# lijrjyan/SDVAR

Measured on AMD Instinct MI355X. Metric: images/s (+ mean accepted tokens/step), VAR-d16 256^2 B=8, d12 draft + d16 verify, per GPU, higher is better.
Workload: dtype f32 (GEMM operands split into 2 fp16 planes to 2^-22, 3 fp16 MFMA products, fp32 accumulate); 1 GPU; BASELINE.json P1: VAR-d16 256^2 B=8/GPU, d12 draft + d16 verify, gamma=2, cfg=1.5 top_k=900 top_p=0.96, acceptance=natural, incl. VQVAE decode (overlapped with the next batch on a 2nd stream); verifier one round behind the draft once gamma = 1; parallelism=1 independent batch shards

## Files before the change

include/sdvar_hip.h:

```cpp
#ifndef SDVAR_HIP_H
#define SDVAR_HIP_H
#include <stdint.h>

#ifdef __cplusplus
extern "C" {
#endif

#define SDVAR_ABI_VERSION 5
#define SDVAR_MAX_STAGES 16

typedef struct sdvar_model sdvar_model_t;
typedef struct sdvar_quant sdvar_quant_t;
typedef struct sdvar_vae sdvar_vae_t;
typedef struct sdvar_vae_enc sdvar_vae_enc_t;

typedef struct {
    int32_t depth;
    int32_t n_stages;
    int32_t patch_nums[SDVAR_MAX_STAGES];
    int32_t vocab;
    int32_t cvae;
    int32_t num_classes;
    int32_t max_batch;
    int32_t max_chunk_stages;
// ... 139 lines not shown
int sdvar_op_quant_nearest(const float* z, int32_t N, const float* codebook, int32_t V, int32_t cvae, float* e2, int64_t* ids, void* stream);
int sdvar_op_conv_planes(const uint16_t* x_planes, uint64_t x_plane_stride, uint64_t x_rows, int32_t x_row0, const uint16_t* w_planes, uint64_t w_plane_stride,
                         int32_t plane_format, const float* w_scale, const float* bias, const float* res, float* out, int32_t B, int32_t H, int32_t W, int32_t N,
                         int32_t Cin, int32_t taps, float* workspace, uint64_t workspace_floats, int32_t force_split, void* stream);
int sdvar_op_conv_planes_ex(const uint16_t* x_planes, uint64_t x_plane_stride, uint64_t x_rows, int32_t x_row0, const uint16_t* w_planes, uint64_t w_plane_stride,
                            int32_t plane_format, const float* w_scale, const float* bias, const float* res, float* out, int32_t B, int32_t H, int32_t W, int32_t N,
                            int32_t Cin, int32_t taps, float* workspace, uint64_t workspace_floats, int32_t force_split, int32_t up_phase, uint64_t w_phase_stride,
                            double* gn_part, float* stats, int32_t* gn_done, void* stream);
int sdvar_op_upconv_weights(const float* w, float* weff, int32_t Cout, int32_t Cin, void* stream);
int sdvar_op_vae_gn_stats(const float* x_rows, int32_t B, int32_t C, int32_t H, int32_t W, double* part_ws, float* stats, void* stream);
int sdvar_op_vae_attn(const float* qkv, float* out, int32_t B, int32_t C, int32_t N, float* workspace, uint64_t ws_floats, int32_t kernel, void* stream);
int sdvar_op_vae_conv_out(const float* x_rows, const float* stats, const float* gamma, const float* beta, const float* w, const float* bias, float* img, int32_t B,
                          int32_t C, int32_t H, int32_t W, float* workspace, void* stream);
int sdvar_debug_set_gemm_cfg(int32_t bm, int32_t split);
int sdvar_debug_set_qkv_fuse(int32_t on);
int sdvar_debug_set_rowblk(int32_t on);
int sdvar_op_gemm_rowblk(const float* x, int32_t ldx, const float* scale, const float* shift, int32_t rows_per_img, int32_t mod_stride, const uint16_t* Xp, uint64_t x_plane_stride,
                         const uint16_t* Wp, uint64_t w_plane_stride, const float* w_scale, const float* bias, float* out, int32_t ldo, uint16_t* out_planes, uint64_t out_plane_stride,
                         int32_t M, int32_t N, int32_t K, int32_t epilogue, const float* res, int32_t ldres, const float* gate, int32_t rows_per_gate, int32_t gate_stride,
                         const float* scale_mul, float* q_out, void* k_cache, void* v_cache, int32_t l, int32_t H, int32_t Lp, int32_t pos0, int32_t kv_fmt, void* stream);
int sdvar_debug_set_variant(const char* name, int32_t value);
int sdvar_debug_get_gemm_cfg(int32_t* out4);
int sdvar_debug_get_conv_cfg(int32_t* out1);
int sdvar_debug_get_conv_plan(int32_t* out4);
int sdvar_debug_plan_gemm(int32_t mode, int32_t M, int32_t N, int32_t K, int32_t flags, int32_t* out4);
int sdvar_debug_set_f16x2_guard(int32_t on);
int sdvar_debug_get_f16x2_guard(uint64_t* out4, int32_t reset);
int sdvar_debug_set_gemm_stamps(uint64_t* stamps);

#define SDVAR_PROF_CLASSES 10
int sdvar_prof_enable(int32_t on);
int sdvar_prof_collect(double* ms , int64_t* launches, double* flops, double* bytes);

int sdvar_op_sdpa_hm(const void* q, const void* k, const void* v, void* out, const int64_t* strides , int32_t dtype , int32_t q_f32,
                     int32_t k_f32, const void* bias, int32_t bias_kind , const int64_t* bias_strides ,
                     const uint8_t* skip_map, int32_t B, int32_t H, int32_t Lq, int32_t Lk, int32_t head_dim, double scale, void* stream);

int sdvar_op_sdpa_hm_lse(const void* q, const void* k, const void* v, void* out, float* lse, const int64_t* strides , int32_t dtype ,
                         int32_t q_f32, int32_t k_f32, const void* bias, int32_t bias_kind ,
                         const int64_t* bias_strides , const uint8_t* skip_map, int32_t B, int32_t H, int32_t Lq, int32_t Lk, int32_t head_dim, double scale,
                         void* stream);
int sdvar_op_sdpa_h_bwd(const void* q, const void* k, const void* v, const void* out, const void* dout, const float* lse, float* delta , void* dq, void* dk,
                        void* dv, const int64_t* strides , int32_t dtype , int32_t q_f32, int32_t k_f32, const void* bias,
                        int32_t bias_kind , const int64_t* bias_strides , const uint8_t* skip_map,
                        int32_t B, int32_t H, int32_t Lq, int32_t Lk, int32_t head_dim, double scale, void* stream);

// ... 66 lines not shown
```

sdvar_amd/csrc/api.hip:

```cpp
#include <math.h>
#include <stdarg.h>
#include <string.h>

#include <vector>

#include "../../include/sdvar_hip.h"
#include "common.h"
#include "gemm_plan.h"

namespace sdvar {

int gemm_f32_nt(const float* X, int ldx, const float* W, const float* bias, float* out, int ldo, int M, int N, int K, int epi,
                const float* res, int ldres, const float* gate, int rows_per_gate, int gate_stride, hipStream_t stream);
struct PendingSplitK { const float* ws; const float* bias; const float* gate; int split, rows_per_gate, gate_stride; };
int ln_modulate(float* x, const float* scale, const float* shift, float* out, uint16_t* outp, size_t ops, int rows, int C, int rows_per_img, int mod_stride, const PendingSplitK* pend, int pfmt, hipStream_t stream);
float* splitk_workspace(size_t* floats);
float* set_splitk_workspace(float* p);
size_t splitk_workspace_floats();
int qk_norm_append(const float* qkv, const float* scale_mul, float* q_out, void* k_cache, void* v_cache, int kv_f16, int R, int l, int H, int Lmax, int pos0, const PendingSplitK* pend, int v_only, hipStream_t stream);
int gemm_f16x2_qkv(const uint16_t* X, size_t xps, const uint16_t* W, size_t wps, const float* wsi, const float* bias, float* out, int ldo, int M, int N, int K,
                   const float* scale_mul, float* q_out, void* k_cache, void* v_cache, int l, int H, int Lp, int pos0, int kv_fmt, int* defer, int* fused, hipStream_t stream);
bool gemm_f16x2_rowblk_ok(int M, int N, int K, int ln, int qkv, bool floor32);
bool gemm_f16x2_rowblk_want(int M, int C, int V, int rows_per_img);
int gemm_f16x2_rowblk(const float* x, int ldx, const float* scale, const float* shift, int rows_per_img, int mod_stride, const uint16_t* X, size_t xps,
// ... 26 lines not shown
int gate_add_bwd(const float* g, const void* y, int ydt, const void* gamma, int gdt, long long gbs, const float* row_scale, void* dy, void* dgamma, int dgamma_rows,
                 float* ws, int B, int L, int C, hipStream_t stream);
long long gate_add_bwd_ws_bytes(int B, int L, int C);
int qknorm_fwd(const void* qkv, int dt, const float* q_bias, const float* v_bias, const float* scale_log, double max_log, float* q, float* k, void* v, int B, int L, int H,
               hipStream_t stream);
int qknorm_bwd(const void* qkv, int dt, const float* q_bias, const float* scale_log, double max_log, const float* dq, const float* dk, const void* dv,
               const long long* strides, void* dqkv, float* dscale_log, float* dq_bias, float* dv_bias, float* ws, int B, int L, int H, hipStream_t stream);
long long qknorm_bwd_ws_bytes(int B, int L, int H);
int cond_lin_fwd(const void* c, int cdt, long long ldc, const void* w, int wdt, const float* b, void* y, int adt, int M, int N, int K, hipStream_t stream);
int cond_lin_bwd(const void* dy, const void* c, int cdt, long long ldc, const void* w, int wdt, void* dc, void* dW, float* db, float* ws, int adt, int M, int N, int K,
                 hipStream_t stream);
long long cond_lin_bwd_ws_bytes(int M, int N, int K);
int embed_fwd(const void* label, int i64, const float* r, double rate, const long long* lvl, const float* xv, long long xbs, long long xrs, const float* class_emb,
              const float* pos_start, const float* W, const float* bias, const float* lvl_emb, const float* pos, void* x, int xdt, float* cond, int B, int T, int L, int first_l,
              int C, int K, int S, int NC1, hipStream_t stream);
int embed_bwd(const void* g, int gdt, const float* gc, const void* label, int i64, const float* r, double rate, const long long* lvl, const float* xv, long long xbs,
              long long xrs, const float* W, float* dpos, float* dpos_start, float* dlvl, float* dclass, float* dbias, float* dW, float* dxv, int xv_rows, float* ws, int B, int T,
              int L, int first_l, int C, int K, int S, int NC1, hipStream_t stream);
long long embed_bwd_ws_bytes(int B, int T, int C, int K);
int optim_grad_stats(const sdvar_optim_tensor_t* ts, int n, const float* grad_scale, const float* found_inf, double max_norm, double beta1, double beta2, void* ws,
                     unsigned long long ws_bytes, hipStream_t stream);
int optim_adamw_step(const sdvar_optim_tensor_t* ts, int n, double beta1, double beta2, double eps, void* ws, unsigned long long ws_bytes, hipStream_t stream);
int attention_f32(const float* q, const void* kc, const void* vc, int kv_f16, float* out, uint16_t* outp, size_t ops, int pfmt, int R, int H, int l, int Lmax, int Ktot, int n_chunk, const int* qbeg, const int* vis, hipStream_t stream);
int gemm_bf16x3_nt(const uint16_t* X, size_t xps, const uint16_t* W, size_t wps, const float* bias, float* out, int ldo, uint16_t* outp, size_t ops,
                   int M, int N, int K, int epi, const float* res, int ldres, const float* gate, int rows_per_gate, int gate_stride, int* defer, hipStream_t stream);
int attention_masked(const float* q, const void* kc, const void* vc, int fmt, const float* bias, float* out, uint16_t* outp, size_t ops, int pfmt, int R, int H, int l,
                     int Lmax, int Ktot, hipStream_t stream);
int attention_sdpa(const float* q, const float* k, const float* v, float* out, const long long* strides, const void* bias, int kind, const long long* bs,
                   const uint8_t* skip, int B, int H, int Lq, int Lk, int head_dim, float scale, hipStream_t stream);
int sdpa_skip_map(const void* bias, int kind, const long long* bs, int Bb, int Hb, int Lq, int Lk, uint8_t* map, hipStream_t stream);
int attention_sdpa_lse(const float* q, const float* k, const float* v, float* out, float* lse, const long long* strides, const void* bias, int kind, const long long* bs,
                       const uint8_t* skip, int B, int H, int Lq, int Lk, int head_dim, float scale, hipStream_t stream);
int attention_sdpa_bwd(const float* q, const float* k, const float* v, const float* out, const float* dout, const float* lse, float* delta, float* dq, float* dk,
                       float* dv, const long long* strides, const void* bias, int kind, const long long* bs, const uint8_t* skip, int B, int H, int Lq, int Lk,
                       int head_dim, float scale, hipStream_t stream);
int attention_sdpa_h(const void* q, const void* k, const void* v, void* out, const long long* strides, int dtype, int B, int H, int Lq, int Lk, int head_dim, double scale,
                     hipStream_t stream);
int attention_sdpa_hm(const void* q, const void* k, const void* v, void* out, const long long* strides, int dtype, int q_f32, int k_f32, const void* bias, int kind,
                      const long long* bs, const uint8_t* skip, int B, int H, int Lq, int Lk, int head_dim, double scale, hipStream_t stream);
int attention_sdpa_hm_lse(const void* q, const void* k, const void* v, void* out, float* lse, const long long* strides, int dtype, int q_f32, int k_f32, const void* bias,
                          int kind, const long long* bs, const uint8_t* skip, int B, int H, int Lq, int Lk, int head_dim, double scale, hipStream_t stream);
int attention_sdpa_h_bwd(const void* q, const void* k, const void* v, const void* out, const void* dout, const float* lse, float* delta, void* dq, void* dk, void* dv,
                         const long long* strides, int dtype, int q_f32, int k_f32, const void* bias, int kind, const long long* bs, const uint8_t* skip, int B, int H,
                         int Lq, int Lk, int head_dim, double scale, hipStream_t stream);
int split_planes(const float* x, uint16_t* planes, int rows, int cols, size_t plane_stride, hipStream_t stream);
int gemm_half_ex(const void* x, const void* w, int dtype, const float* w_scale, const float* bias, float* out, int ldo, void* h_out, void* p_out, const float* res, int ldres,
// ... 1078 lines not shown
int sdvar_debug_plan_gemm(int32_t mode, int32_t M, int32_t N, int32_t K, int32_t flags, int32_t* out4) {
    SDVAR_CHECK_ARG(out4 && mode >= 0 && mode <= 2, "debug_plan_gemm: mode %d", mode);
    SDVAR_CHECK_ARG(M > 0 && N > 0 && K > 0 && K % 32 == 0, "debug_plan_gemm: need K %% 32 == 0 (M=%d N=%d K=%d)", M, N, K);
    const size_t wsf = splitk_workspace_floats();
    const GemmPlan p = mode == 0 ? plan_f32(M, N, K, wsf) : mode == 1 ? plan_bf16x3(M, N, K, wsf) : !(flags & 8) ? plan_f16x2(M, N, K, wsf, flags & 1, flags & 2, flags & 4)
                                                                                                                : plan_f16(M, N, K, wsf, flags & 1, flags & 2, flags & 4);
    out4[0] = p.kernel; out4[1] = p.split; out4[2] = p.tail; out4[3] = p.qkv_fused;
    return SDVAR_OK;
}

int sdvar_debug_get_gemm_cfg(int32_t* out4) {
    SDVAR_CHECK_ARG(out4, "debug_get_gemm_cfg: null");
    int v[4]; debug_get_gemm_cfg_h(v);
    for (int i = 0; i < 4; ++i) out4[i] = v[i];
    return SDVAR_OK;
}

int sdvar_debug_get_conv_cfg(int32_t* out1) {
    SDVAR_CHECK_ARG(out1, "debug_get_conv_cfg: null");
    out1[0] = debug_get_conv_tap_reuse();
    return SDVAR_OK;
}

int sdvar_debug_get_conv_plan(int32_t* out4) {
    SDVAR_CHECK_ARG(out4, "debug_get_conv_plan: null");
    int v[4]; debug_get_conv_plan(v);
    for (int i = 0; i < 4; ++i) out4[i] = v[i];
    return SDVAR_OK;
}

int sdvar_debug_set_f16x2_guard(int32_t on) {
    if (on && !g_guard_cnt) {
        SDVAR_HIP(hipMalloc((void**)&g_guard_cnt, 4 * sizeof(unsigned long long)));
        SDVAR_HIP(hipMemset(g_guard_cnt, 0, 4 * sizeof(unsigned long long)));
    }
    g_guard_on = on != 0;
    return SDVAR_OK;
}

int sdvar_debug_get_f16x2_guard(uint64_t* out4, int32_t reset) {
    SDVAR_CHECK_ARG(out4, "debug_get_f16x2_guard: null");
    for (int i = 0; i < 4; ++i) out4[i] = 0;
    if (!g_guard_cnt) return SDVAR_OK;
    SDVAR_HIP(hipDeviceSynchronize());
    SDVAR_HIP(hipMemcpy(out4, g_guard_cnt, 4 * sizeof(unsigned long long), hipMemcpyDeviceToHost));
    if (reset) SDVAR_HIP(hipMemset(g_guard_cnt, 0, 4 * sizeof(unsigned long long)));
// ... 31 lines not shown
```

sdvar_amd/csrc/attention_f16x2.hip:

```cpp
#include <stdlib.h>

#include "common.h"
#include "gemm_plan.h"

namespace sdvar {

unsigned long long* debug_get_gemm_stamps();

typedef _Float16 f16x8 __attribute__((ext_vector_type(8)));
typedef _Float16 f16x2v __attribute__((ext_vector_type(2)));
typedef uint16_t u16x8 __attribute__((ext_vector_type(8)));
typedef __attribute__((address_space(3))) void* lds_ptr_t;
typedef const __attribute__((address_space(1))) void* glb_ptr_t;

constexpr int ATTH_MAX_CHUNK = 16;
constexpr int AKT = 32;
constexpr int APL = AKT * 64;
constexpr int ANST = 3;

struct AttnHArgs {
    const float* q; const uint16_t* kc; const uint16_t* vc; float* out;
    uint16_t* outp; size_t ops; int pfmt;
    int R, H, l, Lp, Ktot;
    int n_chunk;
    int qbeg[ATTH_MAX_CHUNK + 1];
    int vis[ATTH_MAX_CHUNK];
    unsigned long long* stamps;
};

__device__ __forceinline__ void split8h(const float* v, f16x8& h, f16x8& l) {
#pragma unroll
    for (int e = 0; e < 8; ++e) {
        const float x = clamp_f16_range(v[e]);
        const _Float16 hh = (_Float16)x;
        h[e] = hh; l[e] = (_Float16)(x - (float)hh);
    }
}

typedef short s16x4 __attribute__((ext_vector_type(4)));
__device__ __forceinline__ f16x8 lds_read_tr8(uint32_t addr, int off) {
    typedef __attribute__((address_space(3))) s16x4* lp_t;
    const s16x4 lo = __builtin_amdgcn_ds_read_tr16_b64_v4i16((lp_t)(uintptr_t)(addr + off));
    const s16x4 hi = __builtin_amdgcn_ds_read_tr16_b64_v4i16((lp_t)(uintptr_t)(addr + off + 1024));
    return __builtin_bit_cast(f16x8, __builtin_shufflevector(lo, hi, 0, 1, 2, 3, 4, 5, 6, 7));
}

template <int NKP>
__device__ __forceinline__ void mfma_planes(f32x16& acc, const f16x8* a, const f16x8* b) {
    if (NKP == 2) acc = __builtin_amdgcn_mfma_f32_32x32x16_f16(a[1], b[0], acc, 0, 0, 0);
    acc = __builtin_amdgcn_mfma_f32_32x32x16_f16(a[0], b[1], acc, 0, 0, 0);
// ... 196 lines not shown

    if (wave_active && qi_raw < a.l) {
        const float inv = 1.0f / l_run;
        const size_t obase = ((size_t)r * a.l + qi_raw) * (a.H * 64) + h * 64 + 4 * lh;
#pragma unroll
        for (int g = 0; g < 4; ++g) {
            f32x4 v0, v1;
#pragma unroll
            for (int e = 0; e < 4; ++e) { v0[e] = o0[4 * g + e] * inv; v1[e] = o1[4 * g + e] * inv; }
            if (a.outp) {
                const float u0[4] = {v0[0], v0[1], v0[2], v0[3]}, u1[4] = {v1[0], v1[1], v1[2], v1[3]};
                const int orow = r * a.l + qi_raw, ocol = h * 64 + 4 * lh + 8 * g;
                store_planes4(a.outp, a.ops, kb_index(orow, ocol, a.R * a.l), u0, a.pfmt);
                store_planes4(a.outp, a.ops, kb_index(orow, ocol + 32, a.R * a.l), u1, a.pfmt);
            } else {
                *reinterpret_cast<f32x4*>(a.out + obase + 8 * g) = v0;
                *reinterpret_cast<f32x4*>(a.out + obase + 32 + 8 * g) = v1;
            }
        }
    }
}


template <int NKP, int SCHED>
__global__ __launch_bounds__(512, 2) void attention_f16x2_pp_kernel(AttnHArgs a) {
    extern __shared__ __attribute__((aligned(16))) uint16_t att_sm[];
    constexpr int ASTAGE = 2 * NKP * APL;
    constexpr int PP_NST = SCHED == 0 ? 3 : 2 * SCHED + 2;

    const int tid = threadIdx.x, lane = tid & 63;
    const int wave = __builtin_amdgcn_readfirstlane(tid >> 6);
    const int li = lane & 31, lh = lane >> 5;
    const int qt = blockIdx.x, h = blockIdx.y, r = blockIdx.z;
    const int q0 = qt * 256;
    const int late = wave >> 2;

    const int qi_raw = q0 + wave * 32 + li;
    const int qi = min(qi_raw, a.l - 1);
    int vis_q = a.vis[0];
#pragma unroll 1
    for (int j = 1; j < a.n_chunk; ++j) if (qi >= a.qbeg[j]) vis_q = a.vis[j];
    const int q_last = min(q0 + 255, a.l - 1);
    int kend = a.vis[0];
#pragma unroll 1
    for (int j = 1; j < a.n_chunk; ++j) if (q_last >= a.qbeg[j]) kend = a.vis[j];
    const bool wave_active = (q0 + wave * 32) < a.l;

    f16x8 qp[4][2];
    {
        const float* pq = a.q + (((size_t)r * a.H + h) * a.l + qi) * 64 + 8 * lh;
#pragma unroll
        for (int c = 0; c < 4; ++c) {
            float v[8];
            const f32x4 u0 = *reinterpret_cast<const f32x4*>(pq + 16 * c), u1 = *reinterpret_cast<const f32x4*>(pq + 16 * c + 4);
#pragma unroll
            for (int e = 0; e < 4; ++e) { v[e] = u0[e]; v[4 + e] = u1[e]; }
            split8h(v, qp[c][0], qp[c][1]);
        }
#pragma unroll
        for (int c = 0; c < 4; ++c) { asm volatile("" : "+v"(qp[c][0]), "+v"(qp[c][1])); }
    }

    const size_t head = ((size_t)r * a.H + h) * NKP * (size_t)a.Lp * 64;
    const size_t kps = (size_t)a.Lp * 64;
    const int drow = 8 * (wave & 3) + (lane >> 3);
    const int dchunk = (lane & 7) ^ (late ? 4 * ((drow >> 1) & 1) : ((drow >> 1) & 7));
    const uint32_t ld = (uint32_t)(drow * 64 + 8 * dchunk) * 2u;
    const char* const bsrc = reinterpret_cast<const char*>((late ? a.vc : a.kc) + head);
    const uint32_t lds0 = SDVAR_LDS_ADDR(att_sm);
    auto issue = [&](int t) {
        const uint32_t st = lds0 + (uint32_t)((t % PP_NST) * ASTAGE + (late ? NKP * APL : 0) + (wave & 3) * 512) * 2u;
#pragma unroll
        for (int p = 0; p < NKP; ++p) SDVAR_DMA16(ld, bsrc + (p * kps + (size_t)t * AKT * 64) * 2, st + (uint32_t)(p * APL) * 2u);
    };

    f32x16 o0, o1;
#pragma unroll
    for (int i = 0; i < 16; ++i) { o0[i] = 0.f; o1[i] = 0.f; }
    float M_run = -INFINITY, l_run = 0.f;

    const int swk = (li >> 1) & 7;
    const int vq = (lane >> 2) & 3, vp = lane & 3, vcb = (lane >> 4) & 1;
    const uint32_t koff = (uint32_t)(li * 128), voff0 = (uint32_t)(NKP * APL * 2 + (4 * lh + vq) * 128 + (((vq >> 1) & 1) * 64) + vcb * 32 + vp * 8);
    const int ntiles = (kend + AKT - 1) / AKT;

    f16x8 kf[4][NKP], vf[2][2][NKP];
    auto read_k = [&](int t) {
        const uint32_t sb = lds0 + (uint32_t)((t % PP_NST) * ASTAGE) * 2u;
#pragma unroll
        for (int c = 0; c < 4; ++c)
#pragma unroll
            for (int p = 0; p < NKP; ++p) SDVAR_LDS_RDP(kf[c][p], sb + koff + (uint32_t)(p * APL * 2 + 16 * ((2 * c + lh) ^ swk)));
    };
    auto read_v = [&](int t) {
        const uint32_t sb = lds0 + (uint32_t)((t % PP_NST) * ASTAGE) * 2u;
        const uint32_t sv0 = sb + voff0, sv1 = sv0 ^ 64u;
#pragma unroll
        for (int j = 0; j < 2; ++j)
#pragma unroll
            for (int p = 0; p < NKP; ++p) {
                vf[j][0][p] = lds_read_tr8(sv0, j * 2048 + p * (APL * 2));
                vf[j][1][p] = lds_read_tr8(sv1, j * 2048 + p * (APL * 2));
            }
    };
    auto read_tile = [&](int t) { read_k(t); read_v(t); };
#define SDVAR_PP_SLOT() do { __builtin_amdgcn_sched_barrier(0); __builtin_amdgcn_s_barrier(); __builtin_amdgcn_sched_barrier(0); } while (0)
#ifdef SDVAR_ATT_STAMPS
    unsigned long long stm[5] = {0, 0, 0, 0, 0}, wsr[4] = {0, 0, 0, 0}, wsc[4] = {0, 0, 0, 0};
    wsr[0] = __builtin_amdgcn_s_memrealtime(); wsc[0] = __builtin_amdgcn_s_memtime();
#define SDVAR_PP_STAMP(k) do { if (t == 10) stm[k] = __builtin_amdgcn_s_memtime(); } while (0)
#else
#define SDVAR_PP_STAMP(k) do { } while (0)
#endif

    if constexpr (SCHED >= 1) {
        constexpr int D = PP_NST - 1;
        auto wait_tiles = [&](int n) {
            switch (n * NKP) {
                case 0: asm volatile("s_waitcnt vmcnt(0)" ::: "memory"); break;
                case 1: asm volatile("s_waitcnt vmcnt(1)" ::: "memory"); break;
                case 2: asm volatile("s_waitcnt vmcnt(2)" ::: "memory"); break;
                case 3: asm volatile("s_waitcnt vmcnt(3)" ::: "memory"); break;
                case 4: asm volatile("s_waitcnt vmcnt(4)" ::: "memory"); break;
                case 5: asm volatile("s_waitcnt vmcnt(5)" ::: "memory"); break;
                case 6: asm volatile("s_waitcnt vmcnt(6)" ::: "memory"); break;
                case 8: asm volatile("s_waitcnt vmcnt(8)" ::: "memory"); break;
                case 10: asm volatile("s_waitcnt vmcnt(10)" ::: "memory"); break;
                default: asm volatile("s_waitcnt vmcnt(12)" ::: "memory"); break;
            }
        };
        for (int t = 0; t < D && t < ntiles; ++t) issue(t);
        wait_tiles(min(D, ntiles) - 1);
        SDVAR_PP_SLOT();
        if (late) SDVAR_PP_SLOT();
        read_k(0);
        asm volatile("s_waitcnt lgkmcnt(0)" ::: "memory");
        f16x8 pp[2][2];
#pragma unroll
        for (int j = 0; j < 2; ++j) { pp[j][0] = f16x8{0, 0, 0, 0, 0, 0, 0, 0}; pp[j][1] = pp[j][0]; }
#ifdef SDVAR_ATT_STAMPS
        wsr[1] = __builtin_amdgcn_s_memrealtime(); wsc[1] = __builtin_amdgcn_s_memtime();
// ... 120 lines not shown
                const int orow = r * a.l + qi_raw, ocol = h * 64 + 4 * lh + 8 * g;
                store_planes4(a.outp, a.ops, kb_index(orow, ocol, a.R * a.l), u0, a.pfmt);
                store_planes4(a.outp, a.ops, kb_index(orow, ocol + 32, a.R * a.l), u1, a.pfmt);
            } else {
                *reinterpret_cast<f32x4*>(a.out + obase + 8 * g) = v0;
                *reinterpret_cast<f32x4*>(a.out + obase + 32 + 8 * g) = v1;
            }
        }
    }
#ifdef SDVAR_ATT_STAMPS
    if (a.stamps && blockIdx.x == 0 && blockIdx.y == 0 && blockIdx.z == 0 && lane == 0 && (wave == 0 || wave == 4)) {
        asm volatile("s_waitcnt vmcnt(0)" ::: "memory");
        wsr[3] = __builtin_amdgcn_s_memrealtime(); wsc[3] = __builtin_amdgcn_s_memtime();
#pragma unroll
        for (int k = 0; k < 5; ++k) a.stamps[16 * (wave >> 2) + k] = stm[k];
        if (wave == 0) {
#pragma unroll
            for (int k = 0; k < 4; ++k) { a.stamps[32 + k] = wsr[k]; a.stamps[36 + k] = wsc[k]; }
        }
    }
#endif
}

int attention_f16x2(const float* q, const void* kc, const void* vc, int nkp, float* out, uint16_t* outp, size_t ops, int pfmt, int R, int H, int l, int Lp,
                    int Ktot, int n_chunk, const int* qbeg, const int* vis, hipStream_t stream) {
    SDVAR_CHECK_ARG(q && kc && vc && (out || outp), "attention: null operand");
    SDVAR_CHECK_ARG(nkp == 1 || nkp == 2, "attention: %d cache planes", nkp);
    SDVAR_CHECK_ARG(n_chunk >= 1 && n_chunk <= ATTH_MAX_CHUNK, "attention: chunk of %d stages unsupported (max %d)", n_chunk, ATTH_MAX_CHUNK);
    SDVAR_CHECK_ARG(R > 0 && H > 0 && l > 0 && Ktot >= l && Ktot <= Lp, "attention: bad lengths l=%d Ktot=%d Lmax=%d", l, Ktot, Lp);
    SDVAR_CHECK_ARG(Lp % 64 == 0, "attention: the planes KV formats need Lmax %% 64 == 0 (got %d)", Lp);
    AttnHArgs a;
    a.q = q; a.kc = (const uint16_t*)kc; a.vc = (const uint16_t*)vc; a.out = out; a.outp = outp; a.ops = ops; a.pfmt = pfmt;
    a.R = R; a.H = H; a.l = l; a.Lp = Lp; a.Ktot = Ktot; a.n_chunk = n_chunk;
    for (int j = 0; j < n_chunk; ++j) {
        a.qbeg[j] = qbeg[j]; a.vis[j] = vis[j];
        SDVAR_CHECK_ARG(vis[j] >= 1 && vis[j] <= Ktot && (j == 0 ? qbeg[0] == 0 : (qbeg[j] > qbeg[j - 1] && vis[j] >= vis[j - 1])), "attention: bad stage table at %d", j);
    }
    a.qbeg[n_chunk] = l;
    a.stamps = debug_get_gemm_stamps();
    const size_t lds = ANST * (size_t)(2 * nkp * APL) * sizeof(uint16_t);
    static const int pp_min = getenv("SDVAR_ATTN_PP_MIN") ? atoi(getenv("SDVAR_ATTN_PP_MIN")) : 129;
    const int pp_sched = variant(VAR_ATTN_PP_SCHED);
    if (l >= pp_min) {
        const size_t ldp = (pp_sched == 0 ? 3 : 2 * pp_sched + 2) * (size_t)(2 * nkp * APL) * sizeof(uint16_t);
        const dim3 grid((l + 255) / 256, H, R);
#define SDVAR_PP_LAUNCH(NK, SC) do { static LdsOptIn oi; SDVAR_LDS_OPT_IN(oi, ldp, (const void*)attention_f16x2_pp_kernel<NK, SC>);                         \
                                     hipLaunchKernelGGL((attention_f16x2_pp_kernel<NK, SC>), grid, dim3(512), ldp, stream, a); } while (0)
        switch (pp_sched) {
            case 0: if (nkp == 2) SDVAR_PP_LAUNCH(2, 0); else SDVAR_PP_LAUNCH(1, 0); break;
            case 2: if (nkp == 2) SDVAR_PP_LAUNCH(2, 2); else SDVAR_PP_LAUNCH(1, 2); break;
            case 3: if (nkp == 2) SDVAR_PP_LAUNCH(2, 3); else SDVAR_PP_LAUNCH(1, 3); break;
            default: if (nkp == 2) SDVAR_PP_LAUNCH(2, 1); else SDVAR_PP_LAUNCH(1, 1); break;
        }
#undef SDVAR_PP_LAUNCH
        SDVAR_LAUNCH_CHECK();
        return SDVAR_OK;
    }
    if (nkp == 2) hipLaunchKernelGGL(attention_f16x2_kernel<2>, dim3((l + 127) / 128, H, R), dim3(256), lds, stream, a);
    else hipLaunchKernelGGL(attention_f16x2_kernel<1>, dim3((l + 127) / 128, H, R), dim3(256), lds, stream, a);
    SDVAR_LAUNCH_CHECK();
    return SDVAR_OK;
}

}
```

sdvar_amd/csrc/gemm.hip:

```cpp
#include "common.h"
#include "gemm_plan.h"

namespace sdvar {

enum { EPI_BIAS = 0, EPI_BIAS_GELU = 1, EPI_GATED_RES = 2, EPI_PARTIAL = 3 };

constexpr int BK = 32;
constexpr int LDS_STRIDE = BK + 4;

struct GemmArgs {
    const float* X; const float* W; const float* bias; float* out;
    const float* res; const float* gate;
    int M, N, K, ldx, ldo, ldres;
    int rows_per_gate, gate_stride;
    int split, k_per_split;
};

template <int BM, int BN, int WAVES_M, int WAVES_N, int EPI>
__global__ __launch_bounds__(256) void gemm_f32_nt_kernel(GemmArgs a) {
    static_assert(WAVES_M * WAVES_N == 4, "4 waves per workgroup");
    constexpr int WM = BM / WAVES_M, WN = BN / WAVES_N;
    constexpr int TM = WM / 32, TN = WN / 32;
    static_assert(TM >= 1 && TN >= 1, "wave tile too small");
    constexpr int XV = BM / 32, WV = BN / 32;
// ... 117 lines not shown
        }
    }
}

static thread_local float* g_ws = nullptr;
constexpr size_t WS_FLOATS = (size_t)24 << 20;

static thread_local float* g_ws_model = nullptr;
float* set_splitk_workspace(float* p) { float* old = g_ws_model; g_ws_model = p; return old; }
size_t splitk_workspace_floats() { return WS_FLOATS; }

float* splitk_workspace(size_t* floats) {
    if (floats) *floats = WS_FLOATS;
    if (g_ws_model) return g_ws_model;
    if (!g_ws && hipMalloc((void**)&g_ws, WS_FLOATS * sizeof(float)) != hipSuccess) { set_error("split-K workspace allocation failed"); return nullptr; }
    return g_ws;
}

std::atomic<unsigned> g_variant_epoch{0};
Variant g_variants[VAR_COUNT] = {
    {"gemm_h4_var", "SDVAR_GEMM_H4_VAR", 3, 0, 3, 3, false, false},
    {"gemm_h2_stages", "SDVAR_GEMM_H2_STAGES", 6, 2, 6, 6, false, false},
    {"gemm_small_pp", "SDVAR_GEMM_SMALL_PP", 2, 0, 2, 2, false, false},
    {"attn_pp_sched", "SDVAR_ATTN_PP_SCHED", 1, 0, 3, 1, false, false},
    {"conv_pp", "SDVAR_CONV_PP", 2, 0, 2, 2, true, false},
    {"conv_tap_reuse", "SDVAR_CONV_TAP_REUSE", 1, 0, 1, 1, true, false},
    {"rowblk", "SDVAR_ROWBLK", 1, 0, 2, 1, false, false},
    {"qkv_fuse", "SDVAR_NO_QKV_FUSE", 1, 0, 1, 1, false, true},
    {"gemm_v2", nullptr, 1, 0, 1, 1, false, false},
    {"stage0_table", "SDVAR_STAGE0_TABLE", 1, 0, 1, 1, false, false},
    {"stage0_table_mb", "SDVAR_STAGE0_TABLE_MB", 1024, 0, 1 << 20, 1024, false, false},
    {"h16_min_m", "SDVAR_H16_MIN_M", 2704, 1, 1 << 30, 2704, false, false},
    {nullptr, nullptr, 0, 0, 768, 0, false, false},
    {nullptr, nullptr, 0, -64, 64, 0, false, false},
};

template <int BM, int BN, int WAVES_M, int WAVES_N, int EPI>
static int launch_f32_kernel(const GemmArgs& a, int grid, hipStream_t stream) {
    const size_t lds = 2 * (size_t)(BM + BN) * LDS_STRIDE * sizeof(float);
    static LdsOptIn opt_in;
    SDVAR_LDS_OPT_IN(opt_in, lds, (const void*)gemm_f32_nt_kernel<BM, BN, WAVES_M, WAVES_N, EPI>);
    hipLaunchKernelGGL((gemm_f32_nt_kernel<BM, BN, WAVES_M, WAVES_N, EPI>), dim3(grid), dim3(256), lds, stream, a);
    SDVAR_LAUNCH_CHECK();
    return SDVAR_OK;
}

static int launch_reduce(const GemmArgs& a, const float* ws, int split, int epi, hipStream_t stream) {
// ... 33 lines not shown
```

sdvar_amd/engine.py:

```python
from __future__ import annotations

import contextlib
import ctypes as C
import os
from dataclasses import dataclass, field
from typing import Callable, Dict, List, Optional, Sequence

import numpy as np
import torch

from .ladder import Ladder, as_ladder
from .noise import exponential_noise

_HERE = os.path.dirname(os.path.abspath(__file__))
LIB_PATH = os.path.join(_HERE, "csrc", "libsdvar_hip.so")
MAX_STAGES = 16
ABI_VERSION = 5
GEMM_MODES = ("f32", "bf16x3", "f16x2")
ENGINE_GEMM_MODES = GEMM_MODES + ("f16",)
HALF_KERNEL_CODE = 1128
PLAN_FLAG_F16 = 8
DEFAULT_GEMM_MODE = "f16x2"
PROF_CLASSES = ("gemm", "attention", "ln_modulate", "qk_norm_append", "sampler", "verify", "quant", "embed_misc", "attention_small", "gemm_small")

# ... 113 lines not shown
    "sdvar_op_gate_add_fwd": (_I, [_P, _P, _I, _P, _I, C.c_int64, _P, _P, _I, _I, _I, _P]),
    "sdvar_op_gate_add_bwd_ws_bytes": (C.c_int64, [_I, _I, _I]),
    "sdvar_op_gate_add_bwd": (_I, [_P, _P, _I, _P, _I, C.c_int64, _P, _P, _P, _I, _P, _I, _I, _I, _P]),
    "sdvar_op_qknorm_fwd": (_I, [_P, _I, _P, _P, _P, _D, _P, _P, _P, _I, _I, _I, _P]),
    "sdvar_op_qknorm_bwd_ws_bytes": (C.c_int64, [_I, _I, _I]),
    "sdvar_op_qknorm_bwd": (_I, [_P, _I, _P, _P, _D, _P, _P, _P, _P, _P, _P, _P, _P, _P, _I, _I, _I, _P]),
    "sdvar_op_cond_lin_fwd": (_I, [_P, _I, C.c_int64, _P, _I, _P, _P, _I, _I, _I, _I, _P]),
    "sdvar_op_cond_lin_bwd_ws_bytes": (C.c_int64, [_I, _I, _I]),
    "sdvar_op_cond_lin_bwd": (_I, [_P, _P, _I, C.c_int64, _P, _I, _P, _P, _P, _P, _I, _I, _I, _I, _P]),
    "sdvar_op_embed_fwd": (_I, [_P, _I, _P, _D, _P, _P, C.c_int64, C.c_int64, _P, _P, _P, _P, _P, _P, _P, _I, _P, _I, _I, _I, _I, _I, _I, _I, _I, _P]),
    "sdvar_op_embed_bwd_ws_bytes": (C.c_int64, [_I, _I, _I, _I]),
    "sdvar_op_embed_bwd": (_I, [_P, _I, _P, _P, _I, _P, _D, _P, _P, C.c_int64, C.c_int64, _P, _P, _P, _P, _P, _P, _P, _P, _I, _P, _I, _I, _I, _I, _I, _I, _I, _I, _P]),
    "sdvar_optim_grad_stats": (_I, [_P, _I, _P, _P, _D, _D, _D, _P, _U64, _P]),
    "sdvar_optim_adamw_step": (_I, [_P, _I, _D, _D, _D, _P, _U64, _P]),
    "sdvar_debug_set_gemm_cfg": (_I, [_I, _I]),
    "sdvar_debug_set_gemm_stamps": (_I, [_P]),
    "sdvar_debug_set_qkv_fuse": (_I, [_I]),
    "sdvar_debug_set_rowblk": (_I, [_I]),
    "sdvar_op_gemm_rowblk": (_I, [_P, _I, _P, _P, _I, _I, _P, _U64, _P, _U64, _P, _P, _P, _I, _P, _U64, _I, _I, _I, _I, _P, _I, _P, _I, _I, _P, _P, _P, _P, _I, _I, _I, _I, _I, _P]),
    "sdvar_debug_set_variant": (_I, [C.c_char_p, _I]),
    "sdvar_debug_get_gemm_cfg": (_I, [C.POINTER(_I)]),
    "sdvar_debug_get_conv_cfg": (_I, [C.POINTER(_I)]),
    "sdvar_debug_get_conv_plan": (_I, [C.POINTER(_I)]),
    "sdvar_debug_plan_gemm": (_I, [_I, _I, _I, _I, _I, C.POINTER(_I)]),
    "sdvar_debug_set_f16x2_guard": (_I, [_I]),
    "sdvar_debug_get_f16x2_guard": (_I, [C.POINTER(_U64), _I]),
    "sdvar_prof_enable": (_I, [_I]),
    "sdvar_prof_collect": (_I, [C.POINTER(_D), C.POINTER(C.c_int64), C.POINTER(_D), C.POINTER(_D)]),
}

_lib = None


def load_library(path: str = LIB_PATH):
    global _lib
    if _lib is not None:
        return _lib
    if not os.path.exists(path):
        raise SdvarError(f"{path} not found: build it with `python -c 'import __graft_entry__ as g; g.build()'` "
                         f"(make -C sdvar_amd/csrc); there is no CPU fallback for the sampler")
    lib = C.CDLL(path)
    for name, (res, args) in _SIGNATURES.items():
        fn = getattr(lib, name)
        fn.restype, fn.argtypes = res, args
    if lib.sdvar_abi_version() != ABI_VERSION:
        raise SdvarError("libsdvar_hip.so ABI version mismatch")
# ... 1674 lines not shown
```

Baseline: 193.1 images/s.

## Add 4-wave attention variant with two query rows per lane and make it default

Adds a new attention schedule (SCHED=4) in which a 256-thread block of 4 waves processes 64 query rows per wave, two query groups per lane. Each wave loads both K and V for its own tile slice, and the softmax work of one group is interleaved with the MFMAs of the other using sched_group_barriers. The aim is to reuse each K/V LDS fetch across twice as many queries and to hide softmax latency behind matrix ops. The variant is now the default. It raises register pressure from carrying double accumulators, and the launch skips the LDS opt-in. It also adds timing-experiment hooks and a debug getter that reports which attention path was taken.

```diff
diff --git a/include/sdvar_hip.h b/include/sdvar_hip.h
--- a/include/sdvar_hip.h
+++ b/include/sdvar_hip.h
@@ -185,6 +185,7 @@
 int sdvar_debug_set_variant(const char* name, int32_t value);
 int sdvar_debug_get_gemm_cfg(int32_t* out4);
 int sdvar_debug_get_conv_cfg(int32_t* out1);
+int sdvar_debug_get_attn_cfg(int32_t* out1);
 int sdvar_debug_get_conv_plan(int32_t* out4);
 int sdvar_debug_plan_gemm(int32_t mode, int32_t M, int32_t N, int32_t K, int32_t flags, int32_t* out4);
 int sdvar_debug_set_f16x2_guard(int32_t on);
diff --git a/sdvar_amd/csrc/api.hip b/sdvar_amd/csrc/api.hip
--- a/sdvar_amd/csrc/api.hip
+++ b/sdvar_amd/csrc/api.hip
@@ -72,6 +72,7 @@
                      unsigned long long ws_bytes, hipStream_t stream);
 int optim_adamw_step(const sdvar_optim_tensor_t* ts, int n, double beta1, double beta2, double eps, void* ws, unsigned long long ws_bytes, hipStream_t stream);
 int attention_f32(const float* q, const void* kc, const void* vc, int kv_f16, float* out, uint16_t* outp, size_t ops, int pfmt, int R, int H, int l, int Lmax, int Ktot, int n_chunk, const int* qbeg, const int* vis, hipStream_t stream);
+int debug_get_attn_cfg();
 int gemm_bf16x3_nt(const uint16_t* X, size_t xps, const uint16_t* W, size_t wps, const float* bias, float* out, int ldo, uint16_t* outp, size_t ops,
                    int M, int N, int K, int epi, const float* res, int ldres, const float* gate, int rows_per_gate, int gate_stride, int* defer, hipStream_t stream);
 int attention_masked(const float* q, const void* kc, const void* vc, int fmt, const float* bias, float* out, uint16_t* outp, size_t ops, int pfmt, int R, int H, int l,
@@ -1196,6 +1197,12 @@
     return SDVAR_OK;
 }
 
+int sdvar_debug_get_attn_cfg(int32_t* out1) {
+    SDVAR_CHECK_ARG(out1, "debug_get_attn_cfg: null");
+    out1[0] = debug_get_attn_cfg();
+    return SDVAR_OK;
+}
+
 int sdvar_debug_get_conv_plan(int32_t* out4) {
     SDVAR_CHECK_ARG(out4, "debug_get_conv_plan: null");
     int v[4]; debug_get_conv_plan(v);
diff --git a/sdvar_amd/csrc/attention_f16x2.hip b/sdvar_amd/csrc/attention_f16x2.hip
--- a/sdvar_amd/csrc/attention_f16x2.hip
+++ b/sdvar_amd/csrc/attention_f16x2.hip
@@ -26,6 +26,9 @@
     int qbeg[ATTH_MAX_CHUNK + 1];
     int vis[ATTH_MAX_CHUNK];
     unsigned long long* stamps;
+#ifdef SDVAR_TIMING_EXPERIMENTS
+    int exp_half;
+#endif
 };
 
 __device__ __forceinline__ void split8h(const float* v, f16x8& h, f16x8& l) {
@@ -268,8 +271,230 @@
 }
 
 
+template <int NKP>
+__device__ __forceinline__ void attention_f16x2_w64(const AttnHArgs& a) {
+    extern __shared__ __attribute__((aligned(16))) uint16_t att_sm[];
+    constexpr int ASTAGE = 2 * NKP * APL;
+
+    const int tid = threadIdx.x, lane = tid & 63;
+    const int wave = __builtin_amdgcn_readfirstlane(tid >> 6);
+    const int li = lane & 31, lh = lane >> 5;
+    const int qt = blockIdx.x, h = blockIdx.y, r = blockIdx.z;
+    const int q0 = qt * 256;
+
+    const int qa_raw = q0 + wave * 64 + li, qb_raw = qa_raw + 32;
+    const int qa = min(qa_raw, a.l - 1), qb = min(qb_raw, a.l - 1);
+    int vis_a = a.vis[0], vis_b = a.vis[0];
+#pragma unroll 1
+    for (int j = 1; j < a.n_chunk; ++j) { if (qa >= a.qbeg[j]) vis_a = a.vis[j]; if (qb >= a.qbeg[j]) vis_b = a.vis[j]; }
+    const int q_last = min(q0 + 255, a.l - 1);
+    int kend = a.vis[0];
+#pragma unroll 1
+    for (int j = 1; j < a.n_chunk; ++j) if (q_last >= a.qbeg[j]) kend = a.vis[j];
+    const bool wave_active = (q0 + wave * 64) < a.l;
+
+    f16x8 qpa[4][2], qpb[4][2];
+    {
+        const float* pa = a.q + (((size_t)r * a.H + h) * a.l + qa) * 64 + 8 * lh;
+        const float* pb = a.q + (((size_t)r * a.H + h) * a.l + qb) * 64 + 8 * lh;
+#pragma unroll
+        for (int c = 0; c < 4; ++c) {
+            float v[8], w[8];
+            const f32x4 u0 = *reinterpret_cast<const f32x4*>(pa + 16 * c), u1 = *reinterpret_cast<const f32x4*>(pa + 16 * c + 4);
+            const f32x4 x0 = *reinterpret_cast<const f32x4*>(pb + 16 * c), x1 = *reinterpret_cast<const f32x4*>(pb + 16 * c + 4);
+#pragma unroll
+            for (int e = 0; e < 4; ++e) { v[e] = u0[e]; v[4 + e] = u1[e]; w[e] = x0[e]; w[4 + e] = x1[e]; }
+            split8h(v, qpa[c][0], qpa[c][1]);
+            split8h(w, qpb[c][0], qpb[c][1]);
+        }
+#pragma unroll
+        for (int c = 0; c < 4; ++c) { asm volatile("" : "+v"(qpa[c][0]), "+v"(qpa[c][1]), "+v"(qpb[c][0]), "+v"(qpb[c][1])); }
+    }
+
+    const size_t head = ((size_t)r * a.H + h) * NKP * (size_t)a.Lp * 64;
+    const size_t kps = (size_t)a.Lp * 64;
+    const int krow = 8 * wave + (lane >> 3), kchunk = (lane & 7) ^ ((krow >> 1) & 7), vchunk = (lane & 7) ^ (4 * ((krow >> 1) & 1));
+    const uint32_t lk = (uint32_t)(krow * 64 + 8 * kchunk) * 2u, lv = (uint32_t)(krow * 64 + 8 * vchunk) * 2u;
+    const char* const bk = reinterpret_cast<const char*>(a.kc + head);
+    const char* const bv = reinterpret_cast<const char*>(a.vc + head);
+    auto issue = [&](int t) {
+        uint16_t* st = att_sm + (t % ANST) * ASTAGE + wave * 512;
+#pragma unroll
+        for (int p = 0; p < NKP; ++p) {
+            SDVAR_DMA16(lk, bk + (p * kps + (size_t)t * AKT * 64) * 2, SDVAR_LDS_ADDR(st + p * APL));
+            SDVAR_DMA16(lv, bv + (p * kps + (size_t)t * AKT * 64) * 2, SDVAR_LDS_ADDR(st + (NKP + p) * APL));
+        }
+    };
+
+    f32x16 oa0, oa1, ob0, ob1;
+#pragma unroll
+    for (int i = 0; i < 16; ++i) { oa0[i] = 0.f; oa1[i] = 0.f; ob0[i] = 0.f; ob1[i] = 0.f; }
+    float Ma = -INFINITY, la = 0.f, Mb = -INFINITY, lb = 0.f;
+
+    const int swk = (li >> 1) & 7;
+    const int vq = (lane >> 2) & 3, vp = lane & 3, vcb = (lane >> 4) & 1;
+    const uint32_t voff0 = (uint32_t)((4 * lh + vq) * 128 + (((vq >> 1) & 1) * 64) + vcb * 32 + vp * 8);
+    const int ntiles = (kend + AKT - 1) / AKT;
+    const float L2E = 1.4426950408889634f;
+
+    auto sm_mask = [&](f32x16& s, int k0, int vis_q) {
+        if (__builtin_amdgcn_ballot_w64(k0 + AKT > vis_q) != 0) {
+            asm volatile("" ::: "memory");
+            const int d = vis_q - k0 - 4 * lh;
+#pragma unroll
+            for (int i = 0; i < 16; ++i) if ((i & 3) + 8 * (i >> 2) >= d) s[i] = -INFINITY;
+        }
+    };
+    auto sm_max = [&](const f32x16& s) -> float {
+        float mloc = fmaxf(s[0], s[1]);
+        asm("v_max3_f32 %0, %1, %2, %3" : "=v"(mloc) : "v"(mloc), "v"(s[2]), "v"(s[3]));
+#pragma unroll
+        for (int i = 4; i < 16; i += 2) asm("v_max3_f32 %0, %1, %2, %3" : "=v"(mloc) : "v"(mloc), "v"(s[i]), "v"(s[i + 1]));
+        const auto sw2 = __builtin_amdgcn_permlane32_swap(__float_as_uint(mloc), __float_as_uint(mloc), false, false);
+        mloc = fmaxf(__uint_as_float(sw2[0]), __uint_as_float(sw2[1]));
+        return mloc * L2E;
+    };
+    auto sm_rescale = [&](float mt, float& M_run, float& l_run, f32x16& o0, f32x16& o1) {
+        if (__builtin_amdgcn_ballot_w64(mt > M_run + ATT_DEFER) != 0) {
+            const float M_new = fmaxf(M_run, mt);
+            const float alpha = __builtin_amdgcn_exp2f(M_run - M_new);
+            M_run = M_new;
+            l_run *= alpha;
+#pragma unroll
+            for (int i = 0; i < 16; ++i) { o0[i] *= alpha; o1[i] *= alpha; }
+        }
+    };
+    auto sm_exp = [&](const f32x16& s, float M_run, f32x2 (&pr)[8], f32x2& ls2, int e0, int e1) {
+        const f32x2 l2e2 = {L2E, L2E}, nM2 = {-M_run, -M_run};
+#pragma unroll
+        for (int e = e0; e < e1; ++e) {
+            const f32x2 x = __builtin_elementwise_fma(f32x2{s[2 * e], s[2 * e + 1]}, l2e2, nM2);
+            pr[e] = f32x2{__builtin_amdgcn_exp2f(x[0]), __builtin_amdgcn_exp2f(x[1])};
+            ls2 += pr[e];
+        }
+    };
+    auto sm_sum = [&](const f32x2& ls2, float& l_run) {
+        float lsum = ls2[0] + ls2[1];
+        const auto sw2 = __builtin_amdgcn_permlane32_swap(__float_as_uint(lsum), __float_as_uint(lsum), false, false);
+        lsum = __uint_as_float(sw2[0]) + __uint_as_float(sw2[1]);
+        l_run += lsum;
+    };
+    auto sm_split = [&](const f32x2 (&pr)[8], int j, f16x8 (&pp)[2]) {
+        u32x4 ph, pl;
+#pragma unroll
+        for (int e = 0; e < 4; ++e) {
+            uint32_t hw, lw;
+            split2h_pk_raw(pr[4 * j + e][0], pr[4 * j + e][1], hw, lw);
+            ph[e] = hw; pl[e] = lw;
+        }
+        pp[0] = __builtin_bit_cast(f16x8, ph); pp[1] = __builtin_bit_cast(f16x8, pl);
+    };
+
+    issue(0);
+    if (ntiles > 1) issue(1);
+#pragma unroll 1
+    for (int t = 0; t < ntiles; ++t) {
+        if (t + 1 < ntiles) { if (NKP == 2) asm volatile("s_waitcnt vmcnt(4)" ::: "memory"); else asm volatile("s_waitcnt vmcnt(2)" ::: "memory"); }
+        else asm volatile("s_waitcnt vmcnt(0)" ::: "memory");
+        __builtin_amdgcn_s_barrier();
+        if (t + 2 < ntiles) issue(t + 2);
+        if (!wave_active) continue;
+        const int k0 = t * AKT;
+        const uint16_t* sk = att_sm + (t % ANST) * ASTAGE + li * 64;
+        const uint32_t sv0 = SDVAR_LDS_ADDR(att_sm + (t % ANST) * ASTAGE + NKP * APL) + voff0, sv1 = sv0 ^ 64u;
+        f16x8 kf[4][NKP];
+#pragma unroll
+        for (int c = 0; c < 4; ++c)
+#pragma unroll
+            for (int p = 0; p < NKP; ++p) kf[c][p] = *reinterpret_cast<const f16x8*>(sk + p * APL + 8 * ((2 * c + lh) ^ swk));
+        const f32x16 zero16 = {0.f, 0.f, 0.f, 0.f, 0.f, 0.f, 0.f, 0.f, 0.f, 0.f, 0.f, 0.f, 0.f, 0.f, 0.f, 0.f};
+        f32x16 sa = zero16;
+#pragma unroll
+        for (int c = 0; c < 4; ++c) mfma_planes<NKP>(sa, kf[c], qpa[c]);
+        f16x8 vf[2][2][NKP];
+#pragma unroll
+        for (int j = 0; j < 2; ++j)
+#pragma unroll
+            for (int p = 0; p < NKP; ++p) {
+                vf[j][0][p] = lds_read_tr8(sv0, j * 2048 + p * (APL * 2));
+                vf[j][1][p] = lds_read_tr8(sv1, j * 2048 + p * (APL * 2));
+            }
+#define SDVAR_W64_IL1(NV, ID) __builtin_amdgcn_sched_group_barrier(0x8, 1, ID); __builtin_amdgcn_sched_group_barrier(0x2, NV, ID);
+#define SDVAR_W64_IL(NV, ID) do { SDVAR_W64_IL1(NV, ID) SDVAR_W64_IL1(NV, ID) SDVAR_W64_IL1(NV, ID) SDVAR_W64_IL1(NV, ID) SDVAR_W64_IL1(NV, ID) SDVAR_W64_IL1(NV, ID) \
+                                  __builtin_amdgcn_sched_barrier(0); } while (0)
+        sm_mask(sa, k0, vis_a);
+        __builtin_amdgcn_sched_barrier(0);
+        f32x16 sb = zero16;
+        mfma_planes<NKP>(sb, kf[0], qpb[0]);
+        mfma_planes<NKP>(sb, kf[1], qpb[1]);
+        const float mta = sm_max(sa);
+        SDVAR_W64_IL(3, 1);
+        sm_rescale(mta, Ma, la, oa0, oa1);
+        __builtin_amdgcn_sched_barrier(0);
+        f32x2 pra[8], lsa = {0.f, 0.f};
+        f16x8 ppa[2][2];
+        mfma_planes<NKP>(sb, kf[2], qpb[2]);
+        mfma_planes<NKP>(sb, kf[3], qpb[3]);
+        sm_exp(sa, Ma, pra, lsa, 0, 8);
+        sm_sum(lsa, la);
+        sm_split(pra, 0, ppa[0]);
+        SDVAR_W64_IL(11, 2);
+        sm_mask(sb, k0, vis_b);
+        __builtin_amdgcn_sched_barrier(0);
+        mfma_pv<NKP>(oa0, vf[0][0], ppa[0]);
+        mfma_pv<NKP>(oa1, vf[0][1], ppa[0]);
+        sm_split(pra, 1, ppa[1]);
+        const float mtb = sm_max(sb);
+        SDVAR_W64_IL(6, 3);
+        sm_rescale(mtb, Mb, lb, ob0, ob1);
+        __builtin_amdgcn_sched_barrier(0);
+        f32x2 prb[8], lsb = {0.f, 0.f};
+        f16x8 ppb[2][2];
+        mfma_pv<NKP>(oa0, vf[1][0], ppa[1]);
+        mfma_pv<NKP>(oa1, vf[1][1], ppa[1]);
+        sm_exp(sb, Mb, prb, lsb, 0, 8);
+        sm_sum(lsb, lb);
+        sm_split(prb, 0, ppb[0]);
+        SDVAR_W64_IL(11, 4);
+        mfma_pv<NKP>(ob0, vf[0][0], ppb[0]);
+        mfma_pv<NKP>(ob1, vf[0][1], ppb[0]);
+        sm_split(prb, 1, ppb[1]);
+        SDVAR_W64_IL(4, 5);
+        mfma_pv<NKP>(ob0, vf[1][0], ppb[1]);
+        mfma_pv<NKP>(ob1, vf[1][1], ppb[1]);
+#undef SDVAR_W64_IL
+#undef SDVAR_W64_IL1
+    }
+
+    auto store = [&](int q_raw, float l_run, const f32x16& o0, const f32x16& o1) {
+        if (q_raw >= a.l) return;
+        const float inv = 1.0f / l_run;
+        const size_t obase = ((size_t)r * a.l + q_raw) * (a.H * 64) + h * 64 + 4 * lh;
+#pragma unroll
+        for (int g = 0; g < 4; ++g) {
+            f32x4 v0, v1;
+#pragma unroll
+            for (int e = 0; e < 4; ++e) { v0[e] = o0[4 * g + e] * inv; v1[e] = o1[4 * g + e] * inv; }
+            if (a.outp) {
+                const float u0[4] = {v0[0], v0[1], v0[2], v0[3]}, u1[4] = {v1[0], v1[1], v1[2], v1[3]};
+                const int orow = r * a.l + q_raw, ocol = h * 64 + 4 * lh + 8 * g;
+                store_planes4(a.outp, a.ops, kb_index(orow, ocol, a.R * a.l), u0, a.pfmt);
+                store_planes4(a.outp, a.ops, kb_index(orow, ocol + 32, a.R * a.l), u1, a.pfmt);
+            } else {
+                *reinterpret_cast<f32x4*>(a.out + obase + 8 * g) = v0;
+                *reinterpret_cast<f32x4*>(a.out + obase + 32 + 8 * g) = v1;
+            }
+        }
+    };
+    if (wave_active) {
+        store(qa_raw, la, oa0, oa1);
+        store(qb_raw, lb, ob0, ob1);
+    }
+}
+
 template <int NKP, int SCHED>
-__global__ __launch_bounds__(512, 2) void attention_f16x2_pp_kernel(AttnHArgs a) {
+__global__ __launch_bounds__(SCHED == 4 ? 256 : 512, 2) void attention_f16x2_pp_kernel(AttnHArgs a) {
+    if constexpr (SCHED == 4) { attention_f16x2_w64<NKP>(a); return; }
     extern __shared__ __attribute__((aligned(16))) uint16_t att_sm[];
     constexpr int ASTAGE = 2 * NKP * APL;
     constexpr int PP_NST = SCHED == 0 ? 3 : 2 * SCHED + 2;
@@ -280,6 +505,11 @@
     const int qt = blockIdx.x, h = blockIdx.y, r = blockIdx.z;
     const int q0 = qt * 256;
     const int late = wave >> 2;
+#ifdef SDVAR_TIMING_EXPERIMENTS
+    const bool both = a.exp_half == 2;
+#else
+    constexpr bool both = false;
+#endif
 
     const int qi_raw = q0 + wave * 32 + li;
     const int qi = min(qi_raw, a.l - 1);
@@ -290,7 +520,11 @@
     int kend = a.vis[0];
 #pragma unroll 1
     for (int j = 1; j < a.n_chunk; ++j) if (q_last >= a.qbeg[j]) kend = a.vis[j];
+#ifdef SDVAR_TIMING_EXPERIMENTS
+    const bool wave_active = (q0 + wave * 32) < a.l && !(a.exp_half && late);
+#else
     const bool wave_active = (q0 + wave * 32) < a.l;
+#endif
 
     f16x8 qp[4][2];
     {
@@ -318,6 +552,14 @@
         const uint32_t st = lds0 + (uint32_t)((t % PP_NST) * ASTAGE + (late ? NKP * APL : 0) + (wave & 3) * 512) * 2u;
 #pragma unroll
         for (int p = 0; p < NKP; ++p) SDVAR_DMA16(ld, bsrc + (p * kps + (size_t)t * AKT * 64) * 2, st + (uint32_t)(p * APL) * 2u);
+#ifdef SDVAR_TIMING_EXPERIMENTS
+        if (both) {
+            const uint32_t ldv = (uint32_t)(drow * 64 + 8 * ((lane & 7) ^ (4 * ((drow >> 1) & 1)))) * 2u;
+            const char* const bv = reinterpret_cast<const char*>(a.vc + head);
+#pragma unroll
+            for (int p = 0; p < NKP; ++p) SDVAR_DMA16(ldv, bv + (p * kps + (size_t)t * AKT * 64) * 2, st + (uint32_t)((NKP + p) * APL) * 2u);
+        }
+#endif
     };
 
     f32x16 o0, o1;
@@ -362,7 +604,7 @@
     if constexpr (SCHED >= 1) {
         constexpr int D = PP_NST - 1;
         auto wait_tiles = [&](int n) {
-            switch (n * NKP) {
+            switch (n * NKP * (both ? 2 : 1)) {
                 case 0: asm volatile("s_waitcnt vmcnt(0)" ::: "memory"); break;
                 case 1: asm volatile("s_waitcnt vmcnt(1)" ::: "memory"); break;
                 case 2: asm volatile("s_waitcnt vmcnt(2)" ::: "memory"); break;
@@ -529,6 +771,9 @@
 #endif
 }
 
+static thread_local int g_attn_took = -1;
+int debug_get_attn_cfg() { return g_attn_took; }
+
 int attention_f16x2(const float* q, const void* kc, const void* vc, int nkp, float* out, uint16_t* outp, size_t ops, int pfmt, int R, int H, int l, int Lp,
                     int Ktot, int n_chunk, const int* qbeg, const int* vis, hipStream_t stream) {
     SDVAR_CHECK_ARG(q && kc && vc && (out || outp), "attention: null operand");
@@ -545,14 +790,27 @@
     }
     a.qbeg[n_chunk] = l;
     a.stamps = debug_get_gemm_stamps();
+#ifdef SDVAR_TIMING_EXPERIMENTS
+    a.exp_half = getenv("SDVAR_ATTN_HALF_Q") ? atoi(getenv("SDVAR_ATTN_HALF_Q")) : 0;
+    const int pp_threads = a.exp_half == 2 ? 256 : 512;
+#else
+    constexpr int pp_threads = 512;
+#endif
     const size_t lds = ANST * (size_t)(2 * nkp * APL) * sizeof(uint16_t);
     static const int pp_min = getenv("SDVAR_ATTN_PP_MIN") ? atoi(getenv("SDVAR_ATTN_PP_MIN")) : 129;
     const int pp_sched = variant(VAR_ATTN_PP_SCHED);
+    g_attn_took = l >= pp_min ? 10 + pp_sched : 1;
+    if (l >= pp_min && pp_sched == 4) {
+        if (nkp == 2) hipLaunchKernelGGL((attention_f16x2_pp_kernel<2, 4>), dim3((l + 255) / 256, H, R), dim3(256), lds, stream, a);
+        else hipLaunchKernelGGL((attention_f16x2_pp_kernel<1, 4>), dim3((l + 255) / 256, H, R), dim3(256), lds, stream, a);
+        SDVAR_LAUNCH_CHECK();
+        return SDVAR_OK;
+    }
     if (l >= pp_min) {
         const size_t ldp = (pp_sched == 0 ? 3 : 2 * pp_sched + 2) * (size_t)(2 * nkp * APL) * sizeof(uint16_t);
         const dim3 grid((l + 255) / 256, H, R);
 #define SDVAR_PP_LAUNCH(NK, SC) do { static LdsOptIn oi; SDVAR_LDS_OPT_IN(oi, ldp, (const void*)attention_f16x2_pp_kernel<NK, SC>);                         \
-                                     hipLaunchKernelGGL((attention_f16x2_pp_kernel<NK, SC>), grid, dim3(512), ldp, stream, a); } while (0)
+                                     hipLaunchKernelGGL((attention_f16x2_pp_kernel<NK, SC>), grid, dim3(pp_threads), ldp, stream, a); } while (0)
         switch (pp_sched) {
             case 0: if (nkp == 2) SDVAR_PP_LAUNCH(2, 0); else SDVAR_PP_LAUNCH(1, 0); break;
             case 2: if (nkp == 2) SDVAR_PP_LAUNCH(2, 2); else SDVAR_PP_LAUNCH(1, 2); break;
diff --git a/sdvar_amd/csrc/gemm.hip b/sdvar_amd/csrc/gemm.hip
--- a/sdvar_amd/csrc/gemm.hip
+++ b/sdvar_amd/csrc/gemm.hip
@@ -163,7 +163,7 @@
     {"gemm_h4_var", "SDVAR_GEMM_H4_VAR", 3, 0, 3, 3, false, false},
     {"gemm_h2_stages", "SDVAR_GEMM_H2_STAGES", 6, 2, 6, 6, false, false},
     {"gemm_small_pp", "SDVAR_GEMM_SMALL_PP", 2, 0, 2, 2, false, false},
-    {"attn_pp_sched", "SDVAR_ATTN_PP_SCHED", 1, 0, 3, 1, false, false},
+    {"attn_pp_sched", "SDVAR_ATTN_PP_SCHED", 4, 0, 4, 4, false, false},
     {"conv_pp", "SDVAR_CONV_PP", 2, 0, 2, 2, true, false},
     {"conv_tap_reuse", "SDVAR_CONV_TAP_REUSE", 1, 0, 1, 1, true, false},
     {"rowblk", "SDVAR_ROWBLK", 1, 0, 2, 1, false, false},
diff --git a/sdvar_amd/engine.py b/sdvar_amd/engine.py
--- a/sdvar_amd/engine.py
+++ b/sdvar_amd/engine.py
@@ -159,6 +159,7 @@
     "sdvar_debug_get_gemm_cfg": (_I, [C.POINTER(_I)]),
     "sdvar_debug_get_conv_cfg": (_I, [C.POINTER(_I)]),
     "sdvar_debug_get_conv_plan": (_I, [C.POINTER(_I)]),
+    "sdvar_debug_get_attn_cfg": (_I, [C.POINTER(_I)]),
     "sdvar_debug_plan_gemm": (_I, [_I, _I, _I, _I, _I, C.POINTER(_I)]),
     "sdvar_debug_set_f16x2_guard": (_I, [_I]),
     "sdvar_debug_get_f16x2_guard": (_I, [C.POINTER(_U64), _I]),
```

After: 193.6 images/s, median of 2. No clear change (+0.2%).
